# someone-in-somewhere/multimodal_rag

Hardware: AMD Instinct MI355X
Metric: chunks embedded/sec + queries/sec top_k=5 over 1M×768 at 1/2/4/8 GPUs (higher is better)
Workload: dtype f16

## Files before the change

### multimodal_rag_amd/_native.py

```python
from __future__ import annotations

import ctypes
import os
import threading
from ctypes import c_char_p, c_float, c_int, c_int32, c_int64, c_size_t, c_void_p
from typing import Optional, Tuple

import numpy as np
import torch

_PKG = os.path.dirname(os.path.abspath(__file__))
LIB_PATH = os.path.join(_PKG, "lib", "libmmrag.so")

F32, F16, BF16, F8E4M3 = 0, 1, 2, 3
MAX_K = 20
MAX_K_DEEP = 4096
MAX_MMR_CANDIDATES = 1024
MAX_RESCORE_CANDIDATES = 4096
MAX_GROUP_CANDIDATES, MAX_GROUPS, MAX_GROUP_SIZE = 4096, 256, 16
MAX_FUSE_LISTS, MAX_FUSE_CANDIDATES, MAX_FUSE_RESULTS = 16, 256, 4096
FUSE_METHODS = {"rrf": 0, "max": 1}
MAX_JOIN_PAIRS = 1 << 26
MAX_CLUSTERS = 4096
MAX_SCOPE_GROUPS = 64
# ... 215 lines not shown
    lib.mmrag_encoder_tokens_workspace_bytes.argtypes = [c_void_p, c_int64, c_int, c_int]
    lib.mmrag_encoder_forward_tokens.restype = c_int
    lib.mmrag_encoder_forward_tokens.argtypes = [c_void_p, c_void_p, c_void_p, c_void_p, c_void_p, c_int64, c_int, c_int,
                                                 c_void_p, c_int, c_void_p, c_void_p, c_size_t, c_void_p]
    lib.mmrag_maxsim_scores.restype = c_int
    lib.mmrag_maxsim_scores.argtypes = [c_void_p, c_int64, c_int64, c_void_p, c_int64, c_int64, c_int, c_void_p, c_void_p,
                                        c_int, c_void_p, c_void_p, c_int, c_void_p, c_void_p, c_int, c_void_p, c_void_p,
                                        c_void_p, c_void_p]
    from .lexical import declare as declare_lexical

    declare_lexical(lib)


def lib():
    global _lib
    if _lib is None:
        with _lock:
            if _lib is None:
                if not os.path.exists(LIB_PATH):
                    raise MMRagNativeError(
                        f"{LIB_PATH} is missing: build it with `python -m multimodal_rag_amd.build` "
                        "(hipcc, gfx950).  There is no CPU fallback.")
                handle = ctypes.CDLL(LIB_PATH, mode=ctypes.RTLD_GLOBAL)
                _declare(handle)
                _lib = handle
    return _lib


def _check(status: int, what: str):
    if status != 0:
        msg = lib().mmrag_last_error().decode("utf-8", "replace")
        raise MMRagNativeError(f"{what} failed (status {status}): {msg}")


def _stream_ptr(device) -> int:
    return torch.cuda.current_stream(device).cuda_stream


def _dev_check(*tensors):
    for t in tensors:
        if t is not None and not t.is_cuda:
            raise MMRagNativeError("libmmrag entry points take device (HIP) tensors only; got a CPU tensor")


def _nbytes(t: torch.Tensor) -> int:
    return t.numel() * t.element_size()


def _check_q_rows(who: str, q: torch.Tensor, rows: torch.Tensor, n: Optional[int] = None, other: str = "corpus"):
    if q.dim() != 2 or rows.dim() != 2 or not q.is_contiguous() or not rows.is_contiguous():
        raise MMRagNativeError(f"{who}: q and {other} must be contiguous 2-D tensors")
    if q.dtype != rows.dtype or q.shape[1] != rows.shape[1]:
        raise MMRagNativeError(f"{who}: q and {other} must share dtype and padded width")
    if n is not None and n > rows.shape[0]:
        raise MMRagNativeError(f"{who}: n={n} exceeds corpus capacity {rows.shape[0]}")


def _topk_out(B: int, k: int, device, packed: bool = False) -> Tuple[torch.Tensor, torch.Tensor]:
    if not packed:
        return (torch.empty((B, k), dtype=torch.float32, device=device),
                torch.empty((B, k), dtype=torch.int64, device=device))
    buf = torch.empty(B * k * 12, dtype=torch.uint8, device=device)
    return buf[B * k * 8:].view(torch.float32).view(B, k), buf[: B * k * 8].view(torch.int64).view(B, k)


def search_uses_query_stationary(B: int, n: int, d: int, k: int, dtype: torch.dtype) -> bool:
    return bool(lib().mmrag_internal_search_uses_qs(B, n, padded_dim(d, dtype), _TORCH2DT[dtype], k))


def search_kernel_name(B: int, n: int, d: int, k: int, dtype: torch.dtype) -> str:
    v = lib().mmrag_internal_search_uses_qs(B, n, padded_dim(d, dtype), _TORCH2DT[dtype], k)
    return {0: "cosine_topk_kernel (slab-ring)", 1: "cosine_topk_qs_kernel", 2: "cosine_topk_walk_kernel"}[v]


def padded_dim(d: int, dtype: torch.dtype) -> int:
    v = lib().mmrag_padded_dim(int(d), _TORCH2DT[dtype])
    if v < 0:
        raise MMRagNativeError(f"padded_dim: bad arguments d={d} dtype={dtype}")
    return int(v)


DBG_NO_PREPASS, DBG_8_WAVES, DBG_NO_QS, DBG_FORCE_QS = 1, 2, 4, 8
DBG_OLD_QS, DBG_MFMA32, DBG_MFMA16, DBG_NO_DYN, DBG_NO_SEED = 0x10000, 0x20000, 0x40000, 0x80000, 0x100000


def cosine_topk(q: torch.Tensor, corpus: torch.Tensor, n: int, d: int, k: int, row_offset: int = 0,
                alive_bits: Optional[torch.Tensor] = None,
                workspace: Optional[torch.Tensor] = None, dbg: int = 0,
                packed_out: bool = False) -> Tuple[torch.Tensor, torch.Tensor]:
    _dev_check(q, corpus, alive_bits)
    _check_q_rows("cosine_topk", q, corpus, n)
    B, ld = q.shape
    L = lib()
    need = L.mmrag_cosine_topk_workspace_bytes(B, n, k)
    if workspace is None or _nbytes(workspace) < need:
        workspace = torch.empty(max(need, 16), dtype=torch.uint8, device=q.device)
    out_s, out_r = _topk_out(B, k, q.device, packed_out)
    if dbg:
        cosine_topk_lists(q, corpus, n, d, k, workspace, alive_bits=alive_bits, dbg=dbg)
        return cosine_topk_select(B, n, k, row_offset, workspace, out_s, out_r)
    with torch.cuda.device(q.device):
        st = L.mmrag_cosine_topk(q.data_ptr(), corpus.data_ptr(), B, n, d, ld, _TORCH2DT[q.dtype], k, row_offset,
                                 alive_bits.data_ptr() if alive_bits is not None else None,
                                 out_s.data_ptr(), out_r.data_ptr(), workspace.data_ptr(), _nbytes(workspace),
                                 _stream_ptr(q.device))
    _check(st, "mmrag_cosine_topk")
    return out_s, out_r


DEEP_DBG_NO_BOUND = 1


def cosine_topk_deep(q: torch.Tensor, corpus: torch.Tensor, n: int, d: int, k: int, row_offset: int = 0,
                     alive_bits: Optional[torch.Tensor] = None, workspace: Optional[torch.Tensor] = None,
                     dbg: int = 0, cap: int = 0) -> Tuple[torch.Tensor, torch.Tensor]:
    _dev_check(q, corpus, alive_bits)
    _check_q_rows("cosine_topk_deep", q, corpus, n)
    B, ld = q.shape
    L = lib()
    need = cosine_topk_deep_workspace_bytes(B, n, k)
    if workspace is None or _nbytes(workspace) < need:
        workspace = torch.empty(max(need, 16), dtype=torch.uint8, device=q.device)
    out_s, out_r = _topk_out(B, k, q.device)
    with torch.cuda.device(q.device):
        st = L.mmrag_internal_cosine_topk_deep_ex(
            q.data_ptr(), corpus.data_ptr(), B, n, d, ld, _TORCH2DT[q.dtype], k, row_offset,
            alive_bits.data_ptr() if alive_bits is not None else None, out_s.data_ptr(), out_r.data_ptr(),
            workspace.data_ptr(), _nbytes(workspace), _stream_ptr(q.device), dbg, cap)
    _check(st, "mmrag_cosine_topk_deep")
    return out_s, out_r


def cosine_topk_deep_workspace_bytes(B: int, n: int, k: int) -> int:
    return int(lib().mmrag_cosine_topk_deep_workspace_bytes(B, n, k))


def rescore_topk(q: torch.Tensor, plane: torch.Tensor, d: int, cand_rows: torch.Tensor, k: int,
                 packed_out: bool = False) -> Tuple[torch.Tensor, torch.Tensor]:
    _dev_check(q, plane, cand_rows)
    _check_q_rows("rescore_topk", q, plane, other="plane")
    if cand_rows.dim() != 2 or cand_rows.dtype != torch.int64 or not cand_rows.is_contiguous() \
            or cand_rows.shape[0] != q.shape[0]:
        raise MMRagNativeError("rescore_topk: cand_rows must be a contiguous [B, C] int64 tensor")
    B, C = cand_rows.shape
    out_s, out_r = _topk_out(B, k, q.device, packed_out)
    with torch.cuda.device(q.device):
        st = lib().mmrag_rescore_topk(q.data_ptr(), plane.data_ptr(), plane.shape[1], _TORCH2DT[plane.dtype], d,
                                      cand_rows.data_ptr(), B, C, k, out_s.data_ptr(), out_r.data_ptr(),
                                      _stream_ptr(q.device))
    _check(st, "mmrag_rescore_topk")
    return out_s, out_r


MMR_DBG_STREAM = 1


def mmr_select_workspace_bytes(B: int, C: int, d: int, dtype: torch.dtype) -> int:
    return int(lib().mmrag_mmr_select_workspace_bytes(B, C, d, _TORCH2DT[dtype]))


def mmr_select(corpus: torch.Tensor, d: int, cand_scores: torch.Tensor, cand_rows: torch.Tensor, k: int,
               lambda_mult: float, dbg: int = 0):
    _dev_check(corpus, cand_scores, cand_rows)
    if corpus.dim() != 2 or not corpus.is_contiguous() or corpus.dtype not in _TORCH2DT:
        raise MMRagNativeError("mmr_select: corpus must be a contiguous 2-D tensor of a storage dtype")
    if (cand_scores.dim() != 2 or cand_scores.shape != cand_rows.shape or cand_scores.dtype != torch.float32
# ... 1123 lines not shown
```

### multimodal_rag_amd/csrc/search_qsw.hip

```cpp
#include "search_shared.h"

#include <type_traits>
#include <utility>

using namespace mmrag;

namespace mmrag_impl {

namespace {

template <typename F, int... I>
__device__ __forceinline__ void static_for_impl(F &&f, std::integer_sequence<int, I...>) {
    (f(std::integral_constant<int, I>{}), ...);
}
template <int N, typename F>
__device__ __forceinline__ void static_for(F &&f) {
    static_for_impl(f, std::make_integer_sequence<int, N>{});
}

constexpr int QSW_XCH = 2048 + 64;
constexpr int qsw_lists_bytes(int K, int MS) { return K * (MS == 32 ? 2 : 4) * QS_QROWS * 8; }

constexpr SlabRing qsw_ring(int NK, int K, int MS) {
#if defined(MMRAG_QSW_RING16)
    if (MS == 16 && NK % (MMRAG_QSW_RING16 / 10) == 0) return SlabRing{MMRAG_QSW_RING16 / 10, MMRAG_QSW_RING16 % 10};
#endif
    return slab_ring(NK, qsw_lists_bytes(K, MS) + QSW_XCH);
}

#define MMRAG_QSW_S32(MNEMONIC, QC, C00, C01, C10, C11, ACC)                                                  \
    asm volatile("v_xad_u32 %[t], %[lo], %[xc], %[st]\n\t"                                                    \
                 "ds_read_b128 %[n0], %[t] offset:%[o0]\n\t"                                                  \
                 "ds_read_b128 %[n1], %[t] offset:%[o1]\n\t" MNEMONIC " %[c00], %[a0], %[q0], " C00 "\n\t"    \
                 MNEMONIC " %[c01], %[a0], %[q1], " C01 "\n\t" MNEMONIC " %[c10], %[a1], %[q0], " C10 "\n\t"  \
                 MNEMONIC " %[c11], %[a1], %[q1], " C11 "\n\t"                                                \
                 "s_waitcnt lgkmcnt(0)"                                                                       \
                 : [c00] ACC(c00), [c01] ACC(c01), [c10] ACC(c10), [c11] ACC(c11), [n0] "=&v"(n0),            \
                   [n1] "=&v"(n1), [t] "=&v"(tmp)                                                             \
                 : [a0] "v"(a0), [a1] "v"(a1), [q0] QC(q0), [q1] QC(q1), [lo] "v"(lo), [st] "s"(st),          \
                   [xc] "i"(XC), [o0] "i"(OFF0), [o1] "i"(OFF1))

template <int DT, bool QA, bool FIRST, int XC, int OFF0, int OFF1, typename FT>
__device__ __forceinline__ void qsw_stmt32(f32x16_t &c00, f32x16_t &c01, f32x16_t &c10, f32x16_t &c11, const FT a0,
                                           const FT a1, const FT q0, const FT q1, FT &n0, FT &n1, const unsigned lo,
                                           const unsigned st) {
    unsigned tmp;
    if constexpr (FIRST) {
        static_assert(QA, "the first k-step's Q fragments live in the accumulator file");
        if constexpr (DT == MMRAG_F16) MMRAG_QSW_S32("v_mfma_f32_32x32x16_f16", "a", "0", "0", "0", "0", "=&v");
        else MMRAG_QSW_S32("v_mfma_f32_32x32x16_bf16", "a", "0", "0", "0", "0", "=&v");
    } else if constexpr (DT == MMRAG_F16) {
        if constexpr (QA) MMRAG_QSW_S32("v_mfma_f32_32x32x16_f16", "a", "%[c00]", "%[c01]", "%[c10]", "%[c11]", "+v");
        else MMRAG_QSW_S32("v_mfma_f32_32x32x16_f16", "v", "%[c00]", "%[c01]", "%[c10]", "%[c11]", "+v");
    } else {
        if constexpr (QA) MMRAG_QSW_S32("v_mfma_f32_32x32x16_bf16", "a", "%[c00]", "%[c01]", "%[c10]", "%[c11]", "+v");
        else MMRAG_QSW_S32("v_mfma_f32_32x32x16_bf16", "v", "%[c00]", "%[c01]", "%[c10]", "%[c11]", "+v");
    }
}

#define MMRAG_QSW_S16(MNEMONIC, QC, D0, D1, D2, D3, D4, D5, D6, D7, ACC)                                      \
    asm volatile(MNEMONIC " %[d0], %[a0], %[q0], " D0 "\n\t"                                                  \
                 "ds_read_b128 %[n0], %[ad] offset:%[o0]\n\t" MNEMONIC " %[d1], %[a0], %[q1], " D1 "\n\t"     \
                 "ds_read_b128 %[n1], %[ad] offset:%[o1]\n\t" MNEMONIC " %[d2], %[a0], %[q2], " D2 "\n\t"     \
                 MNEMONIC " %[d3], %[a0], %[q3], " D3 "\n\t" MNEMONIC " %[d4], %[a1], %[q0], " D4 "\n\t"      \
                 MNEMONIC " %[d5], %[a1], %[q1], " D5 "\n\t" MNEMONIC " %[d6], %[a1], %[q2], " D6 "\n\t"      \
                 MNEMONIC " %[d7], %[a1], %[q3], " D7 "\n\t"                                                  \
                 "s_waitcnt lgkmcnt(0)"                                                                       \
                 : [d0] ACC(d0), [d1] ACC(d1), [d2] ACC(d2), [d3] ACC(d3), [d4] ACC(d4), [d5] ACC(d5),        \
                   [d6] ACC(d6), [d7] ACC(d7), [n0] "=&v"(n0), [n1] "=&v"(n1)                                 \
                 : [a0] "v"(a0), [a1] "v"(a1), [q0] QC(q0), [q1] QC(q1), [q2] QC(q2), [q3] QC(q3),            \
                   [ad] "v"(adr), [o0] "i"(OFF0), [o1] "i"(OFF1))
#define MMRAG_QSW_S16_ACC(MNEMONIC, QC)                                                                       \
    MMRAG_QSW_S16(MNEMONIC, QC, "%[d0]", "%[d1]", "%[d2]", "%[d3]", "%[d4]", "%[d5]", "%[d6]", "%[d7]", "+v")
#define MMRAG_QSW_S16_FIRST(MNEMONIC, QC) MMRAG_QSW_S16(MNEMONIC, QC, "0", "0", "0", "0", "0", "0", "0", "0", "=&v")

template <int DT, bool QA, bool FIRST, int OFF0, int OFF1, typename FT>
__device__ __forceinline__ void qsw_stmt16(f32x4_t &d0, f32x4_t &d1, f32x4_t &d2, f32x4_t &d3, f32x4_t &d4,
                                           f32x4_t &d5, f32x4_t &d6, f32x4_t &d7, const FT a0, const FT a1,
                                           const FT q0, const FT q1, const FT q2, const FT q3, FT &n0, FT &n1,
                                           const unsigned adr) {
    if constexpr (FIRST) {
        static_assert(QA, "the first k-step's Q fragments live in the accumulator file");
        if constexpr (DT == MMRAG_F16) MMRAG_QSW_S16_FIRST("v_mfma_f32_16x16x32_f16", "a");
        else MMRAG_QSW_S16_FIRST("v_mfma_f32_16x16x32_bf16", "a");
    } else if constexpr (DT == MMRAG_F16) {
        if constexpr (QA) MMRAG_QSW_S16_ACC("v_mfma_f32_16x16x32_f16", "a");
        else MMRAG_QSW_S16_ACC("v_mfma_f32_16x16x32_f16", "v");
    } else {
        if constexpr (QA) MMRAG_QSW_S16_ACC("v_mfma_f32_16x16x32_bf16", "a");
        else MMRAG_QSW_S16_ACC("v_mfma_f32_16x16x32_bf16", "v");
    }
}

__device__ __forceinline__ void qsw_stage_addr(unsigned &a_lo, unsigned &a_hi, const unsigned lo, const unsigned st) {
    asm volatile("v_add_u32 %0, %2, %3\n\tv_xad_u32 %1, %2, 64, %3" : "=&v"(a_lo), "=&v"(a_hi) : "v"(lo), "s"(st));
}

__device__ __forceinline__ float max16_raw(float x0, float x1, float x2, float x3, float x4, float x5, float x6, float x7,
                                           float x8, float x9, float x10, float x11, float x12, float x13, float x14,
                                           float x15) {
    float r;
    asm("v_max3_f32 %0, %1, %2, %3\n\t"
        "v_max3_f32 %0, %0, %4, %5\n\t"
        "v_max3_f32 %0, %0, %6, %7\n\t"
        "v_max3_f32 %0, %0, %8, %9\n\t"
        "v_max3_f32 %0, %0, %10, %11\n\t"
        "v_max3_f32 %0, %0, %12, %13\n\t"
        "v_max3_f32 %0, %0, %14, %15\n\t"
        "v_max_f32 %0, %0, %16"
        : "=&v"(r)
        : "v"(x0), "v"(x1), "v"(x2), "v"(x3), "v"(x4), "v"(x5), "v"(x6), "v"(x7), "v"(x8), "v"(x9), "v"(x10), "v"(x11),
          "v"(x12), "v"(x13), "v"(x14), "v"(x15));
    return r;
}

constexpr int CP_SC1 = 16;

}

template <int DT, int NK, int K, int MS, bool NT>
__global__ __launch_bounds__(256, 1) void cosine_topk_walk_kernel(const KParams p) {
#if defined(__HIP_DEVICE_COMPILE__)
    using FT = typename FragType<DT>::T;
    static_assert(MS == 32 || MS == 16, "MFMA shape");
    constexpr int R = QS_TILE_ROWS;
    static_assert(R == 64, "statements are written for 64-row tiles");
    constexpr int RB = R / 32;
    constexpr int SLABB = R * SLAB;
    constexpr int NQB = MS == 32 ? 2 : 4;
    constexpr int QW = MS;
    constexpr int NSUB = 64 / QW;
    constexpr int NGRP = 16 / NSUB;
    constexpr SlabRing RING = qsw_ring(NK, K, MS);
    constexpr int G = RING.G, NST = RING.NST;
    constexpr int SPT = NK / G;
    constexpr int STAGE = G * SLABB;
    constexpr int PPS = G * RB;
    constexpr int KSTG = G * 4;
    constexpr int KST = MS == 32 ? NK * 4 : NK * 2;
    constexpr int QA_STEPS = 64 / NQB;
    constexpr int LISTS = qsw_lists_bytes(K, MS);
    constexpr int LOOK = (NST + 1 + SPT - 1) / SPT + 1;
    static_assert(NST >= 3 && NST * STAGE + LISTS + QSW_XCH <= 160 * 1024, "LDS");
    static_assert((NST - 1) * PPS <= 56, "vmcnt range");
    static_assert((G - 1) * SLABB + 48 * SLAB + 2048 < 65536, "ds_read immediate offset");
    static_assert(2 * PPS == KSTG, "one piece after every other statement");
    constexpr int LANDT = ((NST - 2) * PPS + 1 + SPT * PPS - 1) / (SPT * PPS);
    static_assert(LANDT >= 1 && LANDT * SPT * PPS - 1 >= (NST - 2) * PPS, "exchange pieces land before they are used");
    static_assert(LOOK <= 6, "ticket slots");

    __shared__ __attribute__((aligned(1024))) char smem[NST * STAGE + LISTS + QSW_XCH];
    float *lists = (float *)(smem + NST * STAGE);
    float *const gather_lds = (float *)(smem + NST * STAGE + LISTS);
    float *const poll_lds = (float *)(smem + NST * STAGE + LISTS + 1024);
    int *const tk_lds = (int *)(smem + NST * STAGE + LISTS + 2048);

    const int tid = threadIdx.x;
    const int lane = tid & 63;
    const int wave = __builtin_amdgcn_readfirstlane(tid >> 6);
    const int ql = lane & (QW - 1);
    const int sub = lane / QW;
    auto dev_dbg = [&](unsigned flag) -> bool {
#if defined(MMRAG_QSW_DEV)
        return (p.dbg & flag) != 0;
#else
        (void)flag;
        return false;
#endif
    };
    const unsigned long long t_entry = (p.dbg & DBG_QS_CLOCK) ? __builtin_amdgcn_s_memrealtime() : 0ull;

    const unsigned RBy = p.row_bytes;
    const int walkers = p.walkers;
    const int bx = (int)blockIdx.x % walkers;
    const int by = (int)blockIdx.x / walkers;
    const int q0 = by * QS_QROWS;
    const int p_static = p.p_static;
    auto pos_tile = [&](int pos) -> int {
        if (pos < p_static) return bx + pos * walkers;
        return p_static * walkers + (int)((unsigned)__builtin_amdgcn_readfirstlane(tk_lds[pos & 7]) - TICKET0);
    };

    unsigned c_off0;
    {
        const int row = (wave * RB) * 8 + (lane >> 3);
        c_off0 = (unsigned)row * RBy + (unsigned)(((lane & 7) ^ ((row >> 1) & 7)) * 16);
    }
    auto c_off = [&](int i) -> unsigned { return i == 0 ? c_off0 : (c_off0 ^ 64u) + 8u * RBy; };
    int is_pos = 0;
    int fill_tile = bx;
    __amdgpu_buffer_rsrc_t fill_rsrc;
    typedef __attribute__((address_space(3))) char *lds_char_t;
    const lds_char_t wave_lds = (lds_char_t)(lds_ptr_t)(smem + wave * (RB * 1024));
    lds_char_t stage_lds = wave_lds;
    auto fill_open = [&]() {
        const bool real = (unsigned)fill_tile < (unsigned)p.n_tiles && !dev_dbg(DBG_QS_NO_DMA);
        const long long row0 = real ? (dev_dbg(DBG_QS_DMA_L2) ? (long long)bx * R : (long long)fill_tile * R) : 0;
        const long long rows_left = p.n - row0;
        const unsigned c_bytes = real ? (unsigned)((rows_left < R ? rows_left : (long long)R) * (long long)RBy) : 0u;
        fill_rsrc = __builtin_amdgcn_make_buffer_rsrc((void *)(p.corpus + (size_t)row0 * RBy), 0, c_bytes, 0x00020000);
    };
    auto next_fill = [&](auto is_sg_c, int buf) {
        constexpr int IS_SG = decltype(is_sg_c)::value;
        if constexpr (IS_SG == 0) {
            if (is_pos != 0) fill_tile = pos_tile(is_pos);
            fill_open();
            ++is_pos;
        }
        stage_lds = wave_lds + buf * STAGE;
        asm volatile("" : "+s"(stage_lds));
    };
    unsigned koff = 0;
    auto issue_piece = [&](auto is_sg_c, auto pi_c) {
        constexpr int IS_SG = decltype(is_sg_c)::value, PI = decltype(pi_c)::value;
        constexpr int g = PI / RB, i = PI % RB;
        if constexpr (i == 0) asm volatile("s_movk_i32 %0, %1" : "=s"(koff) : "n"((IS_SG * G + g) * SLAB));
        __builtin_amdgcn_raw_ptr_buffer_load_lds(fill_rsrc, (lds_ptr_t)(stage_lds + g * SLABB + i * 1024), 16, c_off(i),
                                                 koff, 0, NT ? 2 : 0);
    };

    const bool any_tile = bx < p.n_tiles;
    if (any_tile)
        static_for<NST>([&](auto st_c) {
            constexpr int st = decltype(st_c)::value;
            next_fill(std::integral_constant<int, st % SPT>{}, st);
            static_for<PPS>([&](auto pi_c) { issue_piece(std::integral_constant<int, st % SPT>{}, pi_c); });
        });
    asm volatile("s_movk_i32 %0, %1" : "=s"(koff) : "n"(((NST - 1) % SPT) * G * SLAB));

    FT qf[NQB][KST];
    float thr[NQB];
    static_for<NQB>([&](auto qb_c) {
        constexpr int qb = decltype(qb_c)::value;
        const int qrow = q0 + wave * 64 + qb * QW + ql;
        const bool live = qrow < p.B;
        const char *src = p.q + (size_t)(live ? qrow : 0) * RBy + sub * 16;
#pragma unroll
        for (int s = 0; s < KST; ++s) {
            FT v = *(const FT *)(src + s * (16 * NSUB));
            if (!live) v = FT{};
            qf[qb][s] = v;
        }
        thr[qb] = !live ? INFINITY : NEG_INF;
    });
    float *const my_lists = lists + tid;
    auto lst_v = [&](int qb, int i) -> float & { return my_lists[(qb * 2 * K + i) * QS_QROWS]; };
    auto lst_r = [&](int qb, int i) -> int & { return *(int *)&my_lists[(qb * 2 * K + K + i) * QS_QROWS]; };
#pragma unroll
    for (int qb = 0; qb < NQB; ++qb)
#pragma unroll
        for (int i = 0; i < K; ++i) {
            lst_v(qb, i) = NEG_INF;
            lst_r(qb, i) = INT_MAX;
        }

    const int sw = (ql >> 1) & 7;
    const unsigned lane_off0 = (unsigned)(ql * SLAB + ((sub ^ sw) * 16));
    const unsigned lane_off64 = lane_off0 ^ 64u;
    const unsigned smem_base = (unsigned)(size_t)(lds_ptr_t)smem;

    auto lane_now = []() -> int {
        int l;
        asm volatile("v_mbcnt_lo_u32_b32 %0, -1, 0\n\tv_mbcnt_hi_u32_b32 %0, -1, %0" : "=v"(l));
        return l;
    };
    f32x16_t c32[MS == 32 ? 4 : 1];
    f32x4_t c16[MS == 16 ? 16 : 1];
    auto score = [&](auto qb_c, auto gi_c, int i) -> float {
        constexpr int qb = decltype(qb_c)::value, gi = decltype(gi_c)::value;
        if constexpr (MS == 32) return c32[(gi >> 2) * 2 + qb][4 * (gi & 3) + i];
        else return c16[gi * 4 + qb][i];
    };
    auto grp_row = [](int gi) -> int { return MS == 32 ? (gi >> 2) * 32 + 8 * (gi & 3) : gi * 16; };
    auto strike = [&](unsigned m0, unsigned m1, const int sub) {
        static_for<NQB>([&](auto qb_c) {
            static_for<NGRP>([&](auto gi_c) {
                constexpr int qb = decltype(qb_c)::value, gi = decltype(gi_c)::value;
                constexpr int r0 = MS == 32 ? (gi >> 2) * 32 + 8 * (gi & 3) : gi * 16;
                const unsigned m = (r0 < 32 ? m0 : m1) >> ((r0 & 31) + 4 * sub);
#pragma unroll
                for (int i = 0; i < 4; ++i) {
                    const bool ok = (m >> i) & 1u;
                    if constexpr (MS == 32) {
                        constexpr int a = (gi >> 2) * 2 + qb, e = 4 * (gi & 3);
                        c32[a][e + i] = ok ? c32[a][e + i] : NEG_INF;
                    } else {
                        c16[gi * 4 + qb][i] = ok ? c16[gi * 4 + qb][i] : NEG_INF;
                    }
                }
            });
        });
    };

    auto select = [&](auto qb_c, const int row_base, float *const my_lists) {
        auto lst_v = [&](int qb, int i) -> float & { return my_lists[(qb * 2 * K + i) * QS_QROWS]; };
        auto lst_r = [&](int qb, int i) -> int & { return *(int *)&my_lists[(qb * 2 * K + K + i) * QS_QROWS]; };
        constexpr int qb = decltype(qb_c)::value;
        auto max16 = [&](auto g0_c) -> float {
            constexpr int g0 = decltype(g0_c)::value;
            using G0 = std::integral_constant<int, g0>;
            using G1 = std::integral_constant<int, g0 + 1>;
            using G2 = std::integral_constant<int, g0 + 2>;
            using G3 = std::integral_constant<int, g0 + 3>;
            return max16_raw(score(qb_c, G0{}, 0), score(qb_c, G0{}, 1), score(qb_c, G0{}, 2), score(qb_c, G0{}, 3),
                             score(qb_c, G1{}, 0), score(qb_c, G1{}, 1), score(qb_c, G1{}, 2), score(qb_c, G1{}, 3),
                             score(qb_c, G2{}, 0), score(qb_c, G2{}, 1), score(qb_c, G2{}, 2), score(qb_c, G2{}, 3),
                             score(qb_c, G3{}, 0), score(qb_c, G3{}, 1), score(qb_c, G3{}, 2), score(qb_c, G3{}, 3));
        };
        float mx = max16(std::integral_constant<int, 0>{});
        if constexpr (NGRP == 8) mx = fmaxf(mx, max16(std::integral_constant<int, 4>{}));
        float t = thr[qb];
        if (__builtin_amdgcn_ballot_w64(mx >= t) == 0ull) return;
        constexpr int NE = NGRP * 4;
        float bar = t;
        if (__builtin_amdgcn_ballot_w64(t == NEG_INF) != 0ull) {
            float prev = INFINITY;
#pragma unroll
            for (int r = 0; r < K; ++r) {
                float m = NEG_INF;
                static_for<NGRP>([&](auto gi_c) {
                    const float x0 = score(qb_c, gi_c, 0), x1 = score(qb_c, gi_c, 1);
                    const float x2 = score(qb_c, gi_c, 2), x3 = score(qb_c, gi_c, 3);
                    const float y0 = x0 < prev ? x0 : NEG_INF, y1 = x1 < prev ? x1 : NEG_INF;
                    const float y2 = x2 < prev ? x2 : NEG_INF, y3 = x3 < prev ? x3 : NEG_INF;
                    m = fmaxf(m, fmaxf(fmaxf(y0, y1), fmaxf(y2, y3)));
                });
                prev = m;
            }
            bar = fmaxf(t, prev);
        }
        unsigned mask = 0;
        static_for<NE>([&](auto e_c) {
            constexpr int e = decltype(e_c)::value;
            mask |= score(qb_c, std::integral_constant<int, e / 4>{}, e % 4) >= bar ? (1u << e) : 0u;
        });
        TopList<K> L;
#pragma unroll
        for (int i = 0; i < K; ++i) {
            L.v[i] = lst_v(qb, i);
            L.r[i] = lst_r(qb, i);
        }
        constexpr int DENSE_AT = NE == 16 ? 8 : 12;
        if (__builtin_amdgcn_ballot_w64(__builtin_popcount(mask) > DENSE_AT) == 0ull) {
            while (__builtin_amdgcn_ballot_w64(mask != 0u) != 0ull) {
                const bool valid = mask != 0u;
                const unsigned e = (unsigned)__builtin_ctz(mask | (1u << (NE - 1)));
                mask &= mask - 1u;
                float lvl[NE];
                static_for<NE>([&](auto e_c) {
                    constexpr int x = decltype(e_c)::value;
                    lvl[x] = score(qb_c, std::integral_constant<int, x / 4>{}, x % 4);
                });
#pragma unroll
                for (int w = NE / 2, b = 0; w >= 1; w >>= 1, ++b) {
                    const bool bit = (e >> b) & 1u;
#pragma unroll
                    for (int i = 0; i < w; ++i) lvl[i] = bit ? lvl[2 * i + 1] : lvl[2 * i];
                }
                const float sc = lvl[0];
                const int row = MS == 32 ? (int)(((e >> 4) << 5) + (((e >> 2) & 3u) << 3) + (e & 3u))
                                         : (int)(((e >> 2) << 4) + (e & 3u));
                L.insert_strict_flat(valid && sc >= t ? sc : NEG_INF, row_base + row);
                t = fmaxf(t, L.v[K - 1]);
            }
        } else {
            static_for<NGRP>([&](auto gi_c) {
                constexpr int gi = decltype(gi_c)::value;
                const float a0 = score(qb_c, gi_c, 0), a1 = score(qb_c, gi_c, 1);
                const float a2 = score(qb_c, gi_c, 2), a3 = score(qb_c, gi_c, 3);
                if (__builtin_amdgcn_ballot_w64(fmaxf(fmaxf(a0, a1), fmaxf(a2, a3)) >= t) != 0ull) {
#pragma clang loop unroll(disable)
                    for (int i = 0; i < 4; ++i) {
                        const float s = i == 0 ? a0 : (i == 1 ? a1 : (i == 2 ? a2 : a3));
                        const bool pass = s >= t;
                        if (__builtin_amdgcn_ballot_w64(pass) != 0ull) {
                            L.insert_strict(pass ? s : NEG_INF, row_base + grp_row(gi) + i);
                            t = fmaxf(t, L.v[K - 1]);
                        }
                    }
                }
            });
        }
        float u = fmaxf(L.v[K - 1], __shfl_xor(L.v[K - 1], QW));
#pragma unroll
        for (int i = 0; i + 1 < K; ++i) u = fmaxf(u, fminf(L.v[i], __shfl_xor(L.v[K - 2 - i], QW)));
        if constexpr (NSUB == 4) u = fmaxf(u, __shfl_xor(u, 32));
        thr[qb] = fmaxf(t, u);
#pragma unroll
        for (int i = 0; i < K; ++i) {
            lst_v(qb, i) = L.v[i];
            lst_r(qb, i) = L.r[i];
        }
    };

    const bool seeding = p.pub_best != nullptr;
    const int n_resp = (QS_QROWS + walkers - 1) / walkers;
    auto publish_bests = [&](const int ql, const int sub, float *const my_lists) {
        auto lst_v = [&](int qb, int i) -> float & { return my_lists[(qb * 2 * K + i) * QS_QROWS]; };
        float *dst = p.pub_best + ((size_t)by * walkers + bx) * QS_QROWS + wave * 64 + ql;
        static_for<NQB>([&](auto qb_c) {
            constexpr int qb = decltype(qb_c)::value;
            float v = lst_v(qb, 0);
            v = fmaxf(v, __shfl_xor(v, QW));
            if constexpr (NSUB == 4) v = fmaxf(v, __shfl_xor(v, 32));
            if (sub == 0) __hip_atomic_store(dst + qb * QW, v, __ATOMIC_RELAXED, __HIP_MEMORY_SCOPE_AGENT);
        });
    };
    auto gather_issue = [&](int q) {
        const int ln = lane_now();
        const __amdgpu_buffer_rsrc_t rs = __builtin_amdgcn_make_buffer_rsrc(
            (void *)(p.pub_best + (size_t)by * walkers * QS_QROWS), 0, (unsigned)(walkers * QS_QROWS * 4), 0x00020000);
#pragma unroll
        for (int c = 0; c < 4; ++c)
            __builtin_amdgcn_raw_ptr_buffer_load_lds(rs, (lds_ptr_t)((char *)gather_lds + c * 256), 4,
                                                     (unsigned)(((c * 64 + ln) * QS_QROWS + q) * 4), 0, 0, CP_SC1);
    };
    auto compute_thr = [&](int q) {
        const int ln = lane_now();
        float v[4];
#pragma unroll
        for (int c = 0; c < 4; ++c) v[c] = (c * 64 + ln) < walkers ? gather_lds[c * 64 + ln] : NEG_INF;
        const float t = wave_kth_largest<K>(v[0], v[1], v[2], v[3], ln);
        if (ln == 0)
            __hip_atomic_store(p.pub_thr + (size_t)by * QS_QROWS + q, t, __ATOMIC_RELAXED, __HIP_MEMORY_SCOPE_AGENT);
    };
    auto poll_issue = [&]() {
        const __amdgpu_buffer_rsrc_t rs = __builtin_amdgcn_make_buffer_rsrc(
            (void *)(p.pub_thr + (size_t)by * QS_QROWS), 0, QS_QROWS * 4, 0x00020000);
        __builtin_amdgcn_raw_ptr_buffer_load_lds(rs, (lds_ptr_t)poll_lds, 16, (unsigned)(lane_now() * 16), 0, 0, CP_SC1);
    };
    auto poll_consume = [&](const int ql) {
        static_for<NQB>([&](auto qb_c) {
            constexpr int qb = decltype(qb_c)::value;
            thr[qb] = fmaxf(thr[qb], poll_lds[wave * 64 + qb * QW + ql]);
        });
    };
    constexpr int STEP = LANDT;
    const int span = n_resp * STEP + LANDT + 1;
    const int pub1 = span + 1 > 5 ? span + 1 : 5;
    auto polled_at = [&](int t) -> bool { return t >= 1 + LANDT && (t < pub1 + span + 4 || (t & 3) == 3); };
    const int quiet = pub1 + span + 4 + LANDT;

    unsigned long long t0c = 0, t0r = 0;
    if (p.dbg & DBG_QS_CLOCK) {
        t0c = __builtin_amdgcn_s_memtime();
        t0r = __builtin_amdgcn_s_memrealtime();
    }
    if (any_tile) {
        FT fa0, fa1, fb0, fb1;
        wait_vmcnt<(NST - 1) * PPS>();
        __builtin_amdgcn_s_barrier();
        {
            const char *st = smem + lane_off0;
            fa0 = *(const FT *)(st);
            fa1 = *(const FT *)(st + (MS == 32 ? 32 * SLAB : 16 * SLAB));
        }
        int cur_tile = bx;
        for (int ti = 0; (unsigned)cur_tile < (unsigned)p.n_tiles; ++ti) {
            unsigned adr_lo = 0, adr_hi = 0;
            if constexpr (MS == 16)
                qsw_stage_addr(adr_lo, adr_hi, lane_off0, smem_base + (unsigned)(((ti * SPT) % NST) * STAGE));
            unsigned tkv;
            const bool want_ticket = ti + LOOK >= p_static && wave == 0;
            if (want_ticket) {
                unsigned long long saved_exec;
                asm volatile("s_mov_b64 %1, exec\n\t"
                             "s_mov_b64 exec, 1\n\t"
                             "global_atomic_add %0, %2, %3, %4 sc0\n\t"
                             "s_mov_b64 exec, %1"
                             : "=&v"(tkv), "=&s"(saved_exec)
                             : "v"(0u), "v"(1u), "s"(p.tickets + by)
                             : "memory");
            }
            static_for<SPT>([&](auto sg_c) {
                constexpr int sg = decltype(sg_c)::value;
                const int it = ti * SPT + sg;
                const unsigned st_cur = smem_base + (unsigned)((it % NST) * STAGE);
                const unsigned st_nxt = smem_base + (unsigned)(((it + 1) % NST) * STAGE);
                static_for<KSTG>([&](auto j_c) {
                    constexpr int j = decltype(j_c)::value;
                    constexpr int g = j / 4, m = j % 4;
                    constexpr bool last = j == KSTG - 1;
                    constexpr int nj = last ? 0 : j + 1;
                    constexpr int ng = nj / 4, nm = nj % 4;
                    constexpr int slab = sg * G + g;
                    const unsigned st = last ? st_nxt : st_cur;
                    FT &x0 = (j & 1) ? fb0 : fa0, &x1 = (j & 1) ? fb1 : fa1;
                    FT &y0 = (j & 1) ? fa0 : fb0, &y1 = (j & 1) ? fa1 : fb1;
                    if constexpr (MS == 32) {
                        constexpr int ks = slab * 4 + m;
                        qsw_stmt32<DT, (ks < QA_STEPS), ks == 0, (nm & 1) * 32, ng * SLABB, ng * SLABB + 32 * SLAB, FT>(
                            c32[0], c32[1], c32[2], c32[3], x0, x1, qf[0][ks], qf[1][ks], y0, y1,
                            (nm & 2) ? lane_off64 : lane_off0, st);
                    } else {
                        constexpr int ks = slab * 2 + (m >> 1), rp = m & 1;
                        constexpr int o0 = ng * SLABB + (nm & 1) * (32 * SLAB);
                        if constexpr (last) qsw_stage_addr(adr_lo, adr_hi, lane_off0, st_nxt);
                        qsw_stmt16<DT, (ks < QA_STEPS), ks == 0, o0, o0 + 16 * SLAB, FT>(
                            c16[rp * 8 + 0], c16[rp * 8 + 1], c16[rp * 8 + 2], c16[rp * 8 + 3], c16[rp * 8 + 4],
                            c16[rp * 8 + 5], c16[rp * 8 + 6], c16[rp * 8 + 7], x0, x1, qf[0][ks], qf[1][ks], qf[2][ks],
                            qf[3][ks], y0, y1, (nm >> 1) ? adr_hi : adr_lo);
                    }
                    if constexpr (j == KSTG - 2) {
                        wait_vmcnt<(NST - 2) * PPS>();
                        if (!dev_dbg(DBG_QS_NO_BARRIER)) __builtin_amdgcn_s_barrier();
                        next_fill(std::integral_constant<int, (NST + sg) % SPT>{}, it % NST);
                    }
                    if constexpr (j == KSTG - 1)
                        issue_piece(std::integral_constant<int, (NST + sg) % SPT>{}, std::integral_constant<int, 0>{});
                    else if constexpr ((j & 1) == 1)
                        issue_piece(std::integral_constant<int, (NST + sg + SPT - 1) % SPT>{},
                                    std::integral_constant<int, (j + 1) / 2>{});
                });
            });
            asm volatile("s_nop 15\n\ts_nop 7");
            const long long row0 = (long long)cur_tile * R;
            if (row0 + R > p.n || p.alive_bits != nullptr) {
                const long long left = p.n - row0;
                unsigned m0 = left >= 32 ? 0xffffffffu : ((1u << (int)left) - 1u);
                unsigned m1 = left >= 64 ? 0xffffffffu : (left > 32 ? ((1u << (int)(left - 32)) - 1u) : 0u);
                if (p.alive_bits != nullptr) {
                    typedef const __attribute__((address_space(4))) uint32_t *scalar_words_t;
                    const scalar_words_t words = (scalar_words_t)p.alive_bits;
                    m0 &= words[row0 >> 5];
                    if (left > 32) m1 &= words[(row0 >> 5) + 1];
                }
                strike(m0, m1, lane_now() / QW);
            }
            const int ln = lane_now();
            const int ql_t = ln & (QW - 1), sub_t = ln / QW;
            float *const lists_t = lists + wave * 64 + ln;
            const int row_base = (int)row0 + 4 * sub_t;
            if (!(p.dbg & DBG_QS_NO_SELECT)) {
                static_for<NQB>([&](auto qb_c) { select(qb_c, row_base, lists_t); });
            } else {
                if constexpr (MS == 32) asm volatile("" ::"v"(c32[0]), "v"(c32[1]), "v"(c32[2]), "v"(c32[3]));
                else {
#pragma unroll
                    for (int e = 0; e < 16; ++e) asm volatile("" ::"v"(c16[e]));
                }
            }
            if (seeding && ti >= quiet) {
                if (((ti - LANDT) & 3) == 3) poll_consume(ql_t);
                if ((ti & 3) == 3 && wave == 0) poll_issue();
            } else if (seeding) {
                if (ti >= LANDT && polled_at(ti - LANDT)) poll_consume(ql_t);
                if (ti == 0 || ti == pub1) publish_bests(ql_t, sub_t, lists_t);
                if (wave == 0) {
                    const int rel = ti > pub1 ? ti - (pub1 + 1) : ti - 1;
                    const int jc = rel - LANDT, jg = rel;
                    if (jc >= 0 && jc % STEP == 0 && jc / STEP < n_resp && bx + (jc / STEP) * walkers < QS_QROWS)
                        compute_thr(bx + (jc / STEP) * walkers);
                    if (jg >= 0 && jg % STEP == 0 && jg / STEP < n_resp && bx + (jg / STEP) * walkers < QS_QROWS)
                        gather_issue(bx + (jg / STEP) * walkers);
                    if (polled_at(ti)) poll_issue();
                }
            }
            if ((p.dbg & DBG_QS_CLOCK) && p.stamps != nullptr && ti < 28 && wave == 0 && ln == 0)
                p.stamps[32 * blockIdx.x + 4 + ti] = __builtin_amdgcn_s_memrealtime();
            if (want_ticket) {
                wait_vmcnt<SPT * PPS>();
                unsigned long long saved_exec;
                const unsigned slot = (unsigned)(size_t)(lds_ptr_t)(tk_lds + ((ti + LOOK) & 7));
                asm volatile("s_mov_b64 %0, exec\n\t"
                             "s_mov_b64 exec, 1\n\t"
                             "ds_write_b32 %1, %2\n\t"
                             "s_mov_b64 exec, %0"
                             : "=&s"(saved_exec)
                             : "v"(slot), "v"(tkv)
                             : "memory");
            }
            cur_tile = pos_tile(ti + 1);
        }
    }
    const int tid_e = wave * 64 + lane_now();
    if ((p.dbg & DBG_QS_CLOCK) && p.stamps != nullptr && tid_e == 0) {
        p.stamps[32 * blockIdx.x] = __builtin_amdgcn_s_memtime() - t0c;
        p.stamps[32 * blockIdx.x + 1] = __builtin_amdgcn_s_memrealtime() - t0r;
        p.stamps[32 * blockIdx.x + 2] = t0r - t_entry;
        p.stamps[32 * blockIdx.x + 3] = t_entry;
    }
    __syncthreads();
    if (q0 + tid_e < p.B) {
        const int w = tid_e >> 6, qb = (tid_e / QW) & (NQB - 1), c = tid_e & (QW - 1);
        const float *la = lists + w * 64 + c + (qb * 2 * K) * QS_QROWS;
        TopList<K> m;
#pragma unroll
        for (int i = 0; i < K; ++i) {
            m.v[i] = la[i * QS_QROWS];
            m.r[i] = __float_as_int(la[(K + i) * QS_QROWS]);
        }
        for (int s = 1; s < NSUB; ++s) {
            const float *lb = la + s * QW;
            for (int i = 0; i < K; ++i) {
                const float x = lb[i * QS_QROWS];
                const int xr = __float_as_int(lb[(K + i) * QS_QROWS]);
                if (xr == INT_MAX || !better(x, xr, m.v[K - 1], m.r[K - 1])) break;
                m.insert_ordered(x, xr);
            }
        }
        const size_t base = ((size_t)(q0 + tid_e) * p.n_lists + bx) * K;
#pragma unroll
        for (int i = 0; i < K; ++i) {
            p.cand_s[base + i] = m.v[i];
            p.cand_r[base + i] = m.r[i];
        }
        if (bx == 0 && p.n_lists > walkers) {
            const size_t seed = ((size_t)(q0 + tid_e) * p.n_lists + (p.n_lists - 1)) * K;
#pragma unroll
            for (int i = 0; i < K; ++i) {
                p.cand_s[seed + i] = NEG_INF;
                p.cand_r[seed + i] = INT_MAX;
            }
        }
    }
#endif
}
// ... 52 lines not shown
```

### multimodal_rag_amd/csrc/search_shared.h

```cpp
#pragma once
#include "mmrag_internal.h"
#include "tile_dma.h"

#include <limits.h>

namespace mmrag_impl {

constexpr float NEG_INF = -__builtin_inff();

__device__ inline bool better(float s, long long r, float s2, long long r2) {
    return s > s2 || (s == s2 && r < r2);
}

template <int K>
struct TopList {
    float v[K];
    int r[K];
    __device__ inline void init() {
#pragma unroll
        for (int i = 0; i < K; ++i) {
            v[i] = NEG_INF;
            r[i] = INT_MAX;
        }
    }
    __device__ inline void insert_ordered(float x, int xr) {
#pragma unroll
        for (int j = 0; j < K; ++j) {
            const bool b = x > v[j] || (x == v[j] && xr < r[j]);
            const float nv = b ? x : v[j];
            const float nx = b ? v[j] : x;
            const int nr = b ? xr : r[j];
            const int nxr = b ? r[j] : xr;
            v[j] = nv;
            x = nx;
            r[j] = nr;
            xr = nxr;
        }
    }
    __device__ inline void insert_strict(float x, int xr) {
#pragma unroll
        for (int j = 0; j < K; ++j) {
            const bool b = x > v[j];
            const float nv = b ? x : v[j];
            const float nx = b ? v[j] : x;
            const int nr = b ? xr : r[j];
            const int nxr = b ? r[j] : xr;
            v[j] = nv;
            x = nx;
            r[j] = nr;
            xr = nxr;
        }
    }
    __device__ inline void insert_strict_flat(float x, int xr) {
        bool c[K];
#pragma unroll
        for (int j = 0; j < K; ++j) c[j] = x > v[j];
#pragma unroll
        for (int j = K - 1; j >= 1; --j) {
            v[j] = c[j] ? (c[j - 1] ? v[j - 1] : x) : v[j];
            r[j] = c[j] ? (c[j - 1] ? r[j - 1] : xr) : r[j];
        }
        v[0] = c[0] ? x : v[0];
        r[0] = c[0] ? xr : r[0];
    }
};

struct KParams {
    const char *q;
    const char *corpus;
    const uint32_t *alive_bits;
    float *cand_s;
    int *cand_r;
    long long n;
    int B;
    unsigned row_bytes;
    int n_tiles;
    int n_lists;
    int tile0;
    int walkers;
    int share_l2;
    const float *thr0;
    unsigned dbg;
    unsigned long long *stamps;
    float *sample_best;
    float *pub_best;
    float *pub_thr;
    unsigned *tickets;
    int p_static;
    int tile_stride;
    unsigned *deep_cnt;
    int deep_cap;
};
constexpr unsigned TICKET0 = 0xff800000u;

constexpr unsigned DBG_QS_NO_SELECT = 16u, DBG_QS_NO_DMA = 32u, DBG_QS_NO_BARRIER = 64u, DBG_QS_DMA_L2 = 512u, DBG_QS_NO_WAIT = 1024u;
constexpr unsigned DBG_QS_CLOCK = 256u;

template <int K>
__device__ inline float wave_kth_largest(float a, float b, float c, float d, int lane) {
    auto ce = [](float &x, float &y) {
        const float hi = fmaxf(x, y), lo = fminf(x, y);
        x = hi;
        y = lo;
    };
    ce(a, b);
    ce(c, d);
    ce(a, c);
    ce(b, d);
    ce(b, c);
    float res = NEG_INF;
    for (int r = 0; r < K; ++r) {
        float m = a;
#pragma unroll
        for (int off = 32; off >= 1; off >>= 1) m = fmaxf(m, __shfl_xor(m, off));
        res = m;
        const unsigned long long owners = __builtin_amdgcn_ballot_w64(a == m);
        if (owners != 0ull && lane == (int)__builtin_ctzll(owners)) {
            a = b;
            b = c;
            c = d;
            d = NEG_INF;
        }
    }
    return res;
}

inline int plan_wn(int B) { return B <= 64 ? 2 : (B <= 128 ? 4 : 8); }
inline int plan_walkers(int tiles, int grid_y) {
    const int cus = mmrag::num_cus();
    int gx = tiles < cus ? tiles : cus;
    if (grid_y > 1 && tiles >= cus) {
        const int w = cus / grid_y / 8 * 8;
        gx = w >= 8 ? w : (cus / grid_y > 0 ? cus / grid_y : 1);
    }
    return gx < 1 ? 1 : gx;
}
int check_search_args(const char *name, int k_max, const void *q, const void *corpus, int B, int64_t n, int d, int64_t ld,
                      int dtype, int k);

bool qs_supported(int dtype, unsigned row_bytes, int K);
constexpr int QS_TILE_ROWS = 64;
constexpr int QS_QROWS = 256;
struct SlabRing {
    int G;
    int NST;
};
constexpr SlabRing slab_ring(int NK, int used_bytes) {
    const int budget = 160 * 1024 - used_bytes;
    for (int need = 4; need >= 3; --need)
        for (int g = 4; g >= 1; --g) {
            if (NK % g) continue;
            int nst = budget / (g * QS_TILE_ROWS * SLAB);
            if (nst > 6) nst = 6;
            if (nst >= need) return SlabRing{g, nst};
        }
    return SlabRing{1, 2};
}
int qs_launch(int dtype, int K, const KParams &p, int grid_x, int grid_y, hipStream_t s);
int qs_seed_thresholds(int K, const float *best, int walkers, int n_queries, float *thr0, hipStream_t s);

constexpr int QSW_DEFAULT_MFMA = 16;
bool qsw_supported(int dtype, unsigned row_bytes, int K, int mfma);
int qsw_launch(int dtype, int K, int mfma, const KParams &p, int grid_x, int grid_y, hipStream_t s);

int deep_filter_launch(int dtype, int WN, const KParams &p, int grid_x, int grid_y, hipStream_t s);

int f8_lists_launch(int K, int WN, const KParams &p, int grid_x, int grid_y, hipStream_t s);
int f8_filter_launch(int WN, const KParams &p, int grid_x, int grid_y, hipStream_t s);


}
```

Baseline: 667,000.

## Rework tile-end top-k selection in walk kernel with parked scores and first-tile fast path

For the 16-wide MFMA path, the per-tile selection is restructured. All four query blocks' max-vs-threshold ballots are computed up front so the whole select is skipped when none fire. The first full tile gets a direct K-round extraction (select_first) that fills lists without an insert loop. Candidate scores are parked in a new LDS region so the sparse insert loop reads them with a pipelined load instead of a mux tree over registers, and the threshold masks are built with hand-written v_cmp/v_addc asm. The extra LDS changes the slab ring sizing, which may reduce pipeline stages, and a debug flag keeps the old tile-end path.

After: 661,300. Within noise of the previous version (-0.9%).

```diff
diff --git a/multimodal_rag_amd/_native.py b/multimodal_rag_amd/_native.py
--- a/multimodal_rag_amd/_native.py
+++ b/multimodal_rag_amd/_native.py
@@ -321,6 +321,7 @@
 
 DBG_NO_PREPASS, DBG_8_WAVES, DBG_NO_QS, DBG_FORCE_QS = 1, 2, 4, 8
 DBG_OLD_QS, DBG_MFMA32, DBG_MFMA16, DBG_NO_DYN, DBG_NO_SEED = 0x10000, 0x20000, 0x40000, 0x80000, 0x100000
+DBG_QS_OLD_TILE_END = 0x400000
 
 
 def cosine_topk(q: torch.Tensor, corpus: torch.Tensor, n: int, d: int, k: int, row_offset: int = 0,
diff --git a/multimodal_rag_amd/csrc/search_qsw.hip b/multimodal_rag_amd/csrc/search_qsw.hip
--- a/multimodal_rag_amd/csrc/search_qsw.hip
+++ b/multimodal_rag_amd/csrc/search_qsw.hip
@@ -20,13 +20,19 @@
 
 constexpr int QSW_XCH = 2048 + 64;
 constexpr int qsw_lists_bytes(int K, int MS) { return K * (MS == 32 ? 2 : 4) * QS_QROWS * 8; }
+constexpr int qsw_park_bytes(int MS) { return MS == 16 ? 16 * 4 * QS_QROWS : 0; }
 
 constexpr SlabRing qsw_ring(int NK, int K, int MS) {
 #if defined(MMRAG_QSW_RING16)
     if (MS == 16 && NK % (MMRAG_QSW_RING16 / 10) == 0) return SlabRing{MMRAG_QSW_RING16 / 10, MMRAG_QSW_RING16 % 10};
 #endif
-    return slab_ring(NK, qsw_lists_bytes(K, MS) + QSW_XCH);
-}
+    return slab_ring(NK, qsw_lists_bytes(K, MS) + QSW_XCH + qsw_park_bytes(MS));
+}
+#if !defined(MMRAG_QSW_RING16)
+static_assert(qsw_ring(12, 5, 16).G == 3 && qsw_ring(12, 5, 16).NST == 4, "ring of 1536-byte rows");
+static_assert(qsw_ring(8, 5, 16).G == 2 && qsw_ring(8, 5, 16).NST == 6, "ring of 1024-byte rows");
+static_assert(qsw_ring(6, 5, 16).G == 3 && qsw_ring(6, 5, 16).NST == 4, "ring of 768-byte rows");
+#endif
 
 #define MMRAG_QSW_S32(MNEMONIC, QC, C00, C01, C10, C11, ACC)                                                  \
     asm volatile("v_xad_u32 %[t], %[lo], %[xc], %[st]\n\t"                                                    \
@@ -113,6 +119,27 @@
           "v"(x12), "v"(x13), "v"(x14), "v"(x15));
     return r;
 }
+
+#define MMRAG_QSW_CMP(OP, X) OP " vcc, " X ", %1\n\tv_addc_co_u32 %0, vcc, %0, %0, vcc\n\t"
+#define MMRAG_QSW_MASK16(NAME, OP)                                                                                      \
+    __device__ __forceinline__ unsigned NAME(float m, float x0, float x1, float x2, float x3, float x4, float x5, float x6, \
+                                             float x7, float x8, float x9, float x10, float x11, float x12, float x13,  \
+                                             float x14, float x15) {                                                    \
+        unsigned r = 0;                                                                                                 \
+        asm(MMRAG_QSW_CMP(OP, "%17") MMRAG_QSW_CMP(OP, "%16") MMRAG_QSW_CMP(OP, "%15") MMRAG_QSW_CMP(OP, "%14")         \
+            MMRAG_QSW_CMP(OP, "%13") MMRAG_QSW_CMP(OP, "%12") MMRAG_QSW_CMP(OP, "%11") MMRAG_QSW_CMP(OP, "%10")         \
+            MMRAG_QSW_CMP(OP, "%9") MMRAG_QSW_CMP(OP, "%8") MMRAG_QSW_CMP(OP, "%7") MMRAG_QSW_CMP(OP, "%6")             \
+            MMRAG_QSW_CMP(OP, "%5") MMRAG_QSW_CMP(OP, "%4") MMRAG_QSW_CMP(OP, "%3") MMRAG_QSW_CMP(OP, "%2")             \
+            : "+v"(r)                                                                                                   \
+            : "v"(m), "v"(x0), "v"(x1), "v"(x2), "v"(x3), "v"(x4), "v"(x5), "v"(x6), "v"(x7), "v"(x8), "v"(x9),         \
+              "v"(x10), "v"(x11), "v"(x12), "v"(x13), "v"(x14), "v"(x15)                                                \
+            : "vcc");                                                                                                   \
+        return r;                                                                                                       \
+    }
+MMRAG_QSW_MASK16(eq_mask16, "v_cmp_eq_f32")
+MMRAG_QSW_MASK16(ge_mask16, "v_cmp_ge_f32")
+#undef MMRAG_QSW_MASK16
+#undef MMRAG_QSW_CMP
 
 constexpr int CP_SC1 = 16;
 
@@ -141,7 +168,8 @@
     constexpr int QA_STEPS = 64 / NQB;
     constexpr int LISTS = qsw_lists_bytes(K, MS);
     constexpr int LOOK = (NST + 1 + SPT - 1) / SPT + 1;
-    static_assert(NST >= 3 && NST * STAGE + LISTS + QSW_XCH <= 160 * 1024, "LDS");
+    constexpr int PARK = qsw_park_bytes(MS);
+    static_assert(NST >= 3 && NST * STAGE + LISTS + QSW_XCH + PARK <= 160 * 1024, "LDS");
     static_assert((NST - 1) * PPS <= 56, "vmcnt range");
     static_assert((G - 1) * SLABB + 48 * SLAB + 2048 < 65536, "ds_read immediate offset");
     static_assert(2 * PPS == KSTG, "one piece after every other statement");
@@ -149,7 +177,7 @@
     static_assert(LANDT >= 1 && LANDT * SPT * PPS - 1 >= (NST - 2) * PPS, "exchange pieces land before they are used");
     static_assert(LOOK <= 6, "ticket slots");
 
-    __shared__ __attribute__((aligned(1024))) char smem[NST * STAGE + LISTS + QSW_XCH];
+    __shared__ __attribute__((aligned(1024))) char smem[NST * STAGE + LISTS + QSW_XCH + PARK];
     float *lists = (float *)(smem + NST * STAGE);
     float *const gather_lds = (float *)(smem + NST * STAGE + LISTS);
     float *const poll_lds = (float *)(smem + NST * STAGE + LISTS + 1024);
@@ -292,10 +320,79 @@
         });
     };
 
-    auto select = [&](auto qb_c, const int row_base, float *const my_lists) {
+    auto with16 = [&](auto qb_c, auto &&f) {
+        using G0 = std::integral_constant<int, 0>;
+        using G1 = std::integral_constant<int, 1>;
+        using G2 = std::integral_constant<int, 2>;
+        using G3 = std::integral_constant<int, 3>;
+        return f(score(qb_c, G0{}, 0), score(qb_c, G0{}, 1), score(qb_c, G0{}, 2), score(qb_c, G0{}, 3),
+                 score(qb_c, G1{}, 0), score(qb_c, G1{}, 1), score(qb_c, G1{}, 2), score(qb_c, G1{}, 3),
+                 score(qb_c, G2{}, 0), score(qb_c, G2{}, 1), score(qb_c, G2{}, 2), score(qb_c, G2{}, 3),
+                 score(qb_c, G3{}, 0), score(qb_c, G3{}, 1), score(qb_c, G3{}, 2), score(qb_c, G3{}, 3));
+    };
+    auto elem_row = [](unsigned e) -> int {
+        return MS == 32 ? (int)(((e >> 4) << 5) + (((e >> 2) & 3u) << 3) + (e & 3u)) : (int)(((e >> 2) << 4) + (e & 3u));
+    };
+    auto round_max = [&](auto qb_c, const float prev) -> float {
+        float m = NEG_INF;
+        static_for<NGRP>([&](auto gi_c) {
+            const float x0 = score(qb_c, gi_c, 0), x1 = score(qb_c, gi_c, 1);
+            const float x2 = score(qb_c, gi_c, 2), x3 = score(qb_c, gi_c, 3);
+            const float y0 = x0 < prev ? x0 : NEG_INF, y1 = x1 < prev ? x1 : NEG_INF;
+            const float y2 = x2 < prev ? x2 : NEG_INF, y3 = x3 < prev ? x3 : NEG_INF;
+            m = fmaxf(m, fmaxf(fmaxf(y0, y1), fmaxf(y2, y3)));
+        });
+        return m;
+    };
+    auto union_bound = [&](const TopList<K> &L) -> float {
+        float u = fmaxf(L.v[K - 1], __shfl_xor(L.v[K - 1], QW));
+#pragma unroll
+        for (int i = 0; i + 1 < K; ++i) u = fmaxf(u, fminf(L.v[i], __shfl_xor(L.v[K - 2 - i], QW)));
+        if constexpr (NSUB == 4) u = fmaxf(u, __shfl_xor(u, 32));
+        return u;
+    };
+    auto select_first = [&](auto qb_c, const int row_base, float *const my_lists) -> bool {
+        constexpr int qb = decltype(qb_c)::value;
+        auto lst_v = [&](int i) -> float & { return my_lists[(qb * 2 * K + i) * QS_QROWS]; };
+        auto lst_r = [&](int i) -> int & { return *(int *)&my_lists[(qb * 2 * K + K + i) * QS_QROWS]; };
+        const float t = thr[qb];
+        const bool live = t == NEG_INF;
+        bool bad = !live && t != INFINITY;
+        float prev = INFINITY;
+#pragma unroll
+        for (int r = 0; r < K; ++r) {
+            const float m = round_max(qb_c, prev);
+            const unsigned eq = with16(qb_c, [&](auto... x) { return eq_mask16(m, x...); });
+            bad |= live && __builtin_popcount(eq) != 1;
+            if (live) {
+                lst_v(r) = m;
+                lst_r(r) = row_base + elem_row((unsigned)__builtin_ctz(eq | 0x8000u));
+            }
+            prev = m;
+        }
+        if (__builtin_amdgcn_ballot_w64(bad) != 0ull) {
+            float ninf;
+            int imax;
+            asm volatile("v_mov_b32 %0, 0xff800000\n\tv_bfrev_b32 %1, -2" : "=v"(ninf), "=v"(imax));
+#pragma unroll
+            for (int i = 0; i < K; ++i) {
+                lst_v(i) = ninf;
+                lst_r(i) = imax;
+            }
+            return false;
+        }
+        TopList<K> L;
+#pragma unroll
+        for (int i = 0; i < K; ++i) L.v[i] = lst_v(i);
+        thr[qb] = fmaxf(fmaxf(t, L.v[K - 1]), union_bound(L));
+        return true;
+    };
+    auto select = [&](auto qb_c, const bool old_end, const int row_base, float *const my_lists, float *const my_park) {
         auto lst_v = [&](int qb, int i) -> float & { return my_lists[(qb * 2 * K + i) * QS_QROWS]; };
         auto lst_r = [&](int qb, int i) -> int & { return *(int *)&my_lists[(qb * 2 * K + K + i) * QS_QROWS]; };
         constexpr int qb = decltype(qb_c)::value;
+        constexpr bool HOISTED = MS == 16;
+        const bool parked_scores = MS == 16 && !old_end;
         auto max16 = [&](auto g0_c) -> float {
             constexpr int g0 = decltype(g0_c)::value;
             using G0 = std::integral_constant<int, g0>;
@@ -307,33 +404,37 @@
                              score(qb_c, G2{}, 0), score(qb_c, G2{}, 1), score(qb_c, G2{}, 2), score(qb_c, G2{}, 3),
                              score(qb_c, G3{}, 0), score(qb_c, G3{}, 1), score(qb_c, G3{}, 2), score(qb_c, G3{}, 3));
         };
-        float mx = max16(std::integral_constant<int, 0>{});
-        if constexpr (NGRP == 8) mx = fmaxf(mx, max16(std::integral_constant<int, 4>{}));
         float t = thr[qb];
-        if (__builtin_amdgcn_ballot_w64(mx >= t) == 0ull) return;
+        if constexpr (!HOISTED) {
+            float mx = max16(std::integral_constant<int, 0>{});
+            if constexpr (NGRP == 8) mx = fmaxf(mx, max16(std::integral_constant<int, 4>{}));
+            if (__builtin_amdgcn_ballot_w64(mx >= t) == 0ull) return;
+        }
         constexpr int NE = NGRP * 4;
         float bar = t;
         if (__builtin_amdgcn_ballot_w64(t == NEG_INF) != 0ull) {
             float prev = INFINITY;
 #pragma unroll
-            for (int r = 0; r < K; ++r) {
-                float m = NEG_INF;
+            for (int r = 0; r < K; ++r) prev = round_max(qb_c, prev);
+            bar = fmaxf(t, prev);
+        }
+        if constexpr (MS == 16) {
+            if (parked_scores)
                 static_for<NGRP>([&](auto gi_c) {
-                    const float x0 = score(qb_c, gi_c, 0), x1 = score(qb_c, gi_c, 1);
-                    const float x2 = score(qb_c, gi_c, 2), x3 = score(qb_c, gi_c, 3);
-                    const float y0 = x0 < prev ? x0 : NEG_INF, y1 = x1 < prev ? x1 : NEG_INF;
-                    const float y2 = x2 < prev ? x2 : NEG_INF, y3 = x3 < prev ? x3 : NEG_INF;
-                    m = fmaxf(m, fmaxf(fmaxf(y0, y1), fmaxf(y2, y3)));
+                    constexpr int gi = decltype(gi_c)::value;
+#pragma unroll
+                    for (int i = 0; i < 4; ++i) my_park[(gi * 4 + i) * QS_QROWS] = c16[gi * 4 + qb][i];
                 });
-                prev = m;
-            }
-            bar = fmaxf(t, prev);
         }
         unsigned mask = 0;
-        static_for<NE>([&](auto e_c) {
-            constexpr int e = decltype(e_c)::value;
-            mask |= score(qb_c, std::integral_constant<int, e / 4>{}, e % 4) >= bar ? (1u << e) : 0u;
-        });
+        if constexpr (MS == 16) {
+            mask = with16(qb_c, [&](auto... x) { return ge_mask16(bar, x...); });
+        } else {
+            static_for<NE>([&](auto e_c) {
+                constexpr int e = decltype(e_c)::value;
+                mask |= score(qb_c, std::integral_constant<int, e / 4>{}, e % 4) >= bar ? (1u << e) : 0u;
+            });
+        }
         TopList<K> L;
 #pragma unroll
         for (int i = 0; i < K; ++i) {
@@ -342,26 +443,43 @@
         }
         constexpr int DENSE_AT = NE == 16 ? 8 : 12;
         if (__builtin_amdgcn_ballot_w64(__builtin_popcount(mask) > DENSE_AT) == 0ull) {
-            while (__builtin_amdgcn_ballot_w64(mask != 0u) != 0ull) {
-                const bool valid = mask != 0u;
-                const unsigned e = (unsigned)__builtin_ctz(mask | (1u << (NE - 1)));
+            if (parked_scores) {
+                auto parked = [&](unsigned e) -> float { return my_park[e * QS_QROWS]; };
+                bool valid = mask != 0u;
+                unsigned e = (unsigned)__builtin_ctz(mask | (1u << (NE - 1)));
                 mask &= mask - 1u;
-                float lvl[NE];
-                static_for<NE>([&](auto e_c) {
-                    constexpr int x = decltype(e_c)::value;
-                    lvl[x] = score(qb_c, std::integral_constant<int, x / 4>{}, x % 4);
-                });
-#pragma unroll
-                for (int w = NE / 2, b = 0; w >= 1; w >>= 1, ++b) {
-                    const bool bit = (e >> b) & 1u;
-#pragma unroll
-                    for (int i = 0; i < w; ++i) lvl[i] = bit ? lvl[2 * i + 1] : lvl[2 * i];
+                float sc = parked(e);
+                while (__builtin_amdgcn_ballot_w64(valid) != 0ull) {
+                    const bool nvalid = mask != 0u;
+                    const unsigned ne = (unsigned)__builtin_ctz(mask | (1u << (NE - 1)));
+                    mask &= mask - 1u;
+                    const float nsc = parked(ne);
+                    L.insert_strict_flat(valid && sc >= t ? sc : NEG_INF, row_base + elem_row(e));
+                    t = fmaxf(t, L.v[K - 1]);
+                    valid = nvalid;
+                    e = ne;
+                    sc = nsc;
                 }
-                const float sc = lvl[0];
-                const int row = MS == 32 ? (int)(((e >> 4) << 5) + (((e >> 2) & 3u) << 3) + (e & 3u))
-                                         : (int)(((e >> 2) << 4) + (e & 3u));
-                L.insert_strict_flat(valid && sc >= t ? sc : NEG_INF, row_base + row);
-                t = fmaxf(t, L.v[K - 1]);
+            } else {
+                while (__builtin_amdgcn_ballot_w64(mask != 0u) != 0ull) {
+                    const bool valid = mask != 0u;
+                    const unsigned e = (unsigned)__builtin_ctz(mask | (1u << (NE - 1)));
+                    mask &= mask - 1u;
+                    float lvl[NE];
+                    static_for<NE>([&](auto e_c) {
+                        constexpr int x = decltype(e_c)::value;
+                        lvl[x] = score(qb_c, std::integral_constant<int, x / 4>{}, x % 4);
+                    });
+#pragma unroll
+                    for (int w = NE / 2, b = 0; w >= 1; w >>= 1, ++b) {
+                        const bool bit = (e >> b) & 1u;
+#pragma unroll
+                        for (int i = 0; i < w; ++i) lvl[i] = bit ? lvl[2 * i + 1] : lvl[2 * i];
+                    }
+                    const float sc = lvl[0];
+                    L.insert_strict_flat(valid && sc >= t ? sc : NEG_INF, row_base + elem_row(e));
+                    t = fmaxf(t, L.v[K - 1]);
+                }
             }
         } else {
             static_for<NGRP>([&](auto gi_c) {
@@ -381,11 +499,7 @@
                 }
             });
         }
-        float u = fmaxf(L.v[K - 1], __shfl_xor(L.v[K - 1], QW));
-#pragma unroll
-        for (int i = 0; i + 1 < K; ++i) u = fmaxf(u, fminf(L.v[i], __shfl_xor(L.v[K - 2 - i], QW)));
-        if constexpr (NSUB == 4) u = fmaxf(u, __shfl_xor(u, 32));
-        thr[qb] = fmaxf(t, u);
+        thr[qb] = fmaxf(t, union_bound(L));
 #pragma unroll
         for (int i = 0; i < K; ++i) {
             lst_v(qb, i) = L.v[i];
@@ -456,6 +570,7 @@
             fa1 = *(const FT *)(st + (MS == 32 ? 32 * SLAB : 16 * SLAB));
         }
         int cur_tile = bx;
+        const bool first_full = p.alive_bits == nullptr && (long long)bx * R + R <= p.n;
         for (int ti = 0; (unsigned)cur_tile < (unsigned)p.n_tiles; ++ti) {
             unsigned adr_lo = 0, adr_hi = 0;
             if constexpr (MS == 16)
@@ -532,7 +647,28 @@
             float *const lists_t = lists + wave * 64 + ln;
             const int row_base = (int)row0 + 4 * sub_t;
             if (!(p.dbg & DBG_QS_NO_SELECT)) {
-                static_for<NQB>([&](auto qb_c) { select(qb_c, row_base, lists_t); });
+                if constexpr (MS == 16) {
+                    unsigned long long fired[NQB];
+                    static_for<NQB>([&](auto qb_c) {
+                        constexpr int qb = decltype(qb_c)::value;
+                        fired[qb] = __builtin_amdgcn_ballot_w64(
+                            with16(qb_c, [&](auto... x) { return max16_raw(x...); }) >= thr[qb]);
+                    });
+                    if ((fired[0] | fired[1] | fired[2] | fired[3]) != 0ull) {
+                        float *const park_t = lists_t + (LISTS + QSW_XCH) / 4;
+                        const bool old_end = (p.dbg & DBG_QS_OLD_TILE_END) != 0;
+                        const bool first = ti == 0 && first_full && !old_end;
+                        static_for<NQB>([&](auto qb_c) {
+                            if (fired[decltype(qb_c)::value] != 0ull) {
+                                bool done = false;
+                                if (first) done = select_first(qb_c, row_base, lists_t);
+                                if (!done) select(qb_c, old_end, row_base, lists_t, park_t);
+                            }
+                        });
+                    }
+                } else {
+                    static_for<NQB>([&](auto qb_c) { select(qb_c, true, row_base, lists_t, nullptr); });
+                }
             } else {
                 if constexpr (MS == 32) asm volatile("" ::"v"(c32[0]), "v"(c32[1]), "v"(c32[2]), "v"(c32[3]));
                 else {
diff --git a/multimodal_rag_amd/csrc/search_shared.h b/multimodal_rag_amd/csrc/search_shared.h
--- a/multimodal_rag_amd/csrc/search_shared.h
+++ b/multimodal_rag_amd/csrc/search_shared.h
@@ -95,6 +95,7 @@
 
 constexpr unsigned DBG_QS_NO_SELECT = 16u, DBG_QS_NO_DMA = 32u, DBG_QS_NO_BARRIER = 64u, DBG_QS_DMA_L2 = 512u, DBG_QS_NO_WAIT = 1024u;
 constexpr unsigned DBG_QS_CLOCK = 256u;
+constexpr unsigned DBG_QS_OLD_TILE_END = 0x400000u;
 
 template <int K>
 __device__ inline float wave_kth_largest(float a, float b, float c, float d, int lane) {
```
